# jjhbw/GoMILP

Measured on AMD Instinct MI355X. Metric: simplex pivots/sec on 2048x4096 fp64 dense LP, higher is better.
Workload: dtype f64

## Files before the change

gomilp_amd/csrc/lu_cross.hip:

```cpp
#include <hip/hip_runtime.h>
#include <stdint.h>

#include "bt_loop.h"
#include "device_types.h"
#include "kernels_common.h"
#include "luc_role.h"

namespace gomilp {

namespace {

constexpr int kLxSlots = 24;
constexpr int kLxSlots32 = 40;
constexpr int kLxHeader = 16;
constexpr int kLxSpinLimit = 400000;

__device__ __forceinline__ void lx_load3(const xpair *p0, const xpair *p1, const xpair *p2, xpair (&v)[3]) {
    asm volatile("global_load_dwordx4 %0, %3, off sc1\n\tglobal_load_dwordx4 %1, %4, off sc1\n\tglobal_load_dwordx4 %2, %5, off sc1\n\ts_waitcnt vmcnt(0)"
                 : "=&v"(v[0]), "=&v"(v[1]), "=&v"(v[2]) : "v"(p0), "v"(p1), "v"(p2) : "memory");
}

__device__ __forceinline__ void lx_load3_fast(const xpair *p0, const xpair *p1, const xpair *p2, xpair (&v)[3]) {
    asm volatile("global_load_dwordx4 %0, %3, off nt\n\tglobal_load_dwordx4 %1, %4, off nt\n\tglobal_load_dwordx4 %2, %5, off nt\n\ts_waitcnt vmcnt(0)"
                 : "=&v"(v[0]), "=&v"(v[1]), "=&v"(v[2]) : "v"(p0), "v"(p1), "v"(p2) : "memory");
}

__device__ __forceinline__ void lx_load5(const xpair *p, xpair (&v)[5]) {
    asm volatile("global_load_dwordx4 %0, %5, off sc1\n\tglobal_load_dwordx4 %1, %5, off offset:128 sc1\n\tglobal_load_dwordx4 %2, %5, off offset:256 sc1\n\t"
                 "global_load_dwordx4 %3, %5, off offset:384 sc1\n\tglobal_load_dwordx4 %4, %5, off offset:512 sc1\n\ts_waitcnt vmcnt(0)"
                 : "=&v"(v[0]), "=&v"(v[1]), "=&v"(v[2]), "=&v"(v[3]), "=&v"(v[4]) : "v"(p) : "memory");
}
__device__ __forceinline__ void lx_load5_fast(const xpair *p, xpair (&v)[5]) {
    asm volatile("global_load_dwordx4 %0, %5, off nt\n\tglobal_load_dwordx4 %1, %5, off offset:128 nt\n\tglobal_load_dwordx4 %2, %5, off offset:256 nt\n\t"
                 "global_load_dwordx4 %3, %5, off offset:384 nt\n\tglobal_load_dwordx4 %4, %5, off offset:512 nt\n\ts_waitcnt vmcnt(0)"
                 : "=&v"(v[0]), "=&v"(v[1]), "=&v"(v[2]), "=&v"(v[3]), "=&v"(v[4]) : "v"(p) : "memory");
}

}

#ifdef GOMILP_DEBUG
__device__ unsigned long long g_lux_stamps[4 * 16];
#define LUX_STAMP(S)                                                                      \
    do {                                                                                  \
        unsigned long long t_;                                                            \
        __builtin_amdgcn_sched_barrier(0);                                                \
        asm volatile("s_memtime %0\n\ts_waitcnt lgkmcnt(0)" : "=s"(t_)::"memory");        \
        __builtin_amdgcn_sched_barrier(0);                                                \
        if ((S) >= 0) tacc[(S) >= 0 ? (S) : 0] += t_ - tprev;                             \
        tprev = t_;                                                                       \
    } while (0)
#else
#define LUX_STAMP(S) do { } while (0)
#endif

template <int G, int RPT, int NB, int SMAX, bool LK>
__global__ __launch_bounds__(256) void k_luc_panel_x(LUArgs a, int32_t *__restrict__ pivrow, xpair *__restrict__ xrec) {
    constexpr int T = 256, NW = 4, MAXM = 256 * RPT * G;
    static_assert((NB == 16 || NB == 32) && SMAX <= 32 && G <= 8, "register tuples of 16 slots; lane l polls record l >> 3");
    static_assert(RPT == 1 || ((RPT == 4 || RPT == 8) && G == 8), "several rows per lane: the eight-workgroup panel");
    static_assert(!LK || RPT == 1, "the look-ahead role: one row per lane");
    static_assert(RPT < 8 || NB == 16, "eight rows per lane: one tuple of 16 slots");
    static_assert(MAXM <= 16384, "rows below 16384 fit (cnt << 16) | row in redL");
    constexpr bool KEEPX = RPT <= 4;
    constexpr int NH = NB / 16;
    constexpr int NSL = NB == 16 ? kLxSlots : kLxSlots32;
    constexpr int NLD = NSL / 8;
    constexpr int NUSE = 5 + NB;
    typedef unsigned short idx_t;
    typedef double vec __attribute__((ext_vector_type(16)));
    constexpr idx_t NONE = 0xFFFF;
    const int bx = (int)blockIdx.x;
    if ((bx & 7) || (bx >> 3) >= G) {
        if constexpr (LK) {
            if (!a.ctl_base->fault) luc_role<T, SMAX, true>(a, bx - min(G, (bx + 7) >> 3), (int)gridDim.x - G);
        }
        return;
    }
    const int g = bx >> 3;
    __shared__ idx_t s_lpos[MAXM];
    __shared__ idx_t s_rowat[MAXM];
    __shared__ idx_t s_unit[MAXM];
    __shared__ idx_t s_ucol[MAXM];
    __shared__ unsigned char s_active[MAXM];
    __shared__ double redM[2][NW];
    __shared__ unsigned int redL[2][NW];
    __shared__ int s_slotcol[NB];
    __shared__ int s_nload, s_stop, s_limit, s_sigma;
    __shared__ __attribute__((aligned(16))) double s_post[NW][NSL];
    if (a.ctl_base->fault) return;
    LUCtl *ctl = a.ctl;
    const int tid = threadIdx.x, lane = tid & 63, w = tid >> 6;
    const int m = a.m;
    const size_t ldw = (size_t)a.ldw;
    const int k0 = a.ctl_prev->k_next;
    if (k0 >= m) {
        if (g == 0 && tid == 0) luc_ctl_empty(ctl, a.ctl_prev, k0, true);
        return;
    }
#ifdef GOMILP_DEBUG
    unsigned long long tacc[16] = {}, tprev = 0;
#endif
    LUX_STAMP(-1);
    for (int R = tid; R < MAXM; R += T) {
        const bool in = R < m;
        s_lpos[R] = (idx_t)(in ? a.lpos[R] : R);
        s_active[R] = (in && a.rowstep[R] < 0) ? 1 : 0;
        const int ur = (in && a.unit_row) ? a.unit_row[R] : -1;
        s_unit[R] = ur < 0 ? NONE : (idx_t)ur;
        s_ucol[R] = NONE;
    }
    __syncthreads();
    for (int R = tid; R < m; R += T) {
        s_rowat[s_lpos[R]] = (idx_t)R;
        if (s_unit[R] != NONE && R >= k0) s_ucol[s_unit[R]] = (idx_t)R;
    }
    for (;;) {
        __syncthreads();
        bool again = false;
        for (int R = tid; R < m; R += T)
            if (s_unit[R] != NONE && R >= k0 && R < (int)s_ucol[s_unit[R]]) { s_ucol[s_unit[R]] = (idx_t)R; again = true; }
        if (!__syncthreads_or(again)) break;
    }
    if (w == 0) {
        const int n = luc_scan_dense<NB>(k0, m, s_unit, s_active, s_slotcol);
        if (lane == 0) s_nload = n;
    }
    __syncthreads();
    const int nload = s_nload;
    int myslotcol = (lane < NB && lane < nload) ? s_slotcol[lane < NB ? lane : 0] : 0x7FFFFFFF;
    int myslotin = -1;
    unsigned int live = nload >= 32 ? 0xFFFFFFFFu : ((1u << nload) - 1u);
    const int R0 = g * (T * RPT) + tid;
    bool act[RPT];
    int myucol[RPT];
#pragma unroll
    for (int r = 0; r < RPT; r++) {
        const int R = R0 + T * r;
        act[r] = (R < m) && s_active[R < m ? R : 0];
        const idx_t uc0 = s_ucol[R < m ? R : 0];
        myucol[r] = (act[r] && uc0 != NONE) ? (int)uc0 : 0x7FFFFFFF;
    }
    LUX_STAMP(9);
    if constexpr (LK) {
        if (tid == 0) s_stop = luc_spin(&a.ctl_base->cnt_u, (uint32_t)(a.round + 1) * (uint32_t)((m + 63) / 64)) ? 1 : 0;
        __syncthreads();
        if (!s_stop) {
            if (tid == 0) {
                a.ctl_base->fault = 1;
                if (g == 0) luc_ctl_empty(ctl, a.ctl_prev, k0, true);
            }
            return;
        }
    }
    LUX_STAMP(10);
    vec v[RPT][NH];
#pragma unroll
    for (int r = 0; r < RPT; r++) {
        const double *src = a.W + (act[r] ? R0 + T * r : 0);
        if constexpr (LK) {
#pragma unroll
            for (int c = 0; c < NB; c++) v[r][c / 16][c % 16] = (act[r] && c < nload) ? luc_ld_agent(&src[(size_t)__builtin_amdgcn_readlane(myslotcol, c) * ldw]) : 0.0;
        } else {
#pragma unroll
            for (int c = 0; c < NB; c++) v[r][c / 16][c % 16] = (act[r] && c < nload) ? src[(size_t)__builtin_amdgcn_readlane(myslotcol, c) * ldw] : 0.0;
        }
    }
    __syncthreads();
    __builtin_amdgcn_s_waitcnt(0x0F70);
    unsigned int myxcc;
    asm volatile("s_getreg_b32 %0, hwreg(HW_REG_XCC_ID)" : "=s"(myxcc));
    myxcc &= 0xFu;
    bool fast = false;
    const double seq0 = xrec[0][0];
    xpair *recs = xrec + kLxHeader / 2;
    int nx = 0;
    LUX_STAMP(11);
    int kcur = k0, s = 0, k1 = m;
    int ksync = a.ctl_prev->ksync;
    bool fault = false;
#pragma unroll 1
    for (;;) {
        if (w == 0) {
            const unsigned int key = (lane < NB && ((live >> lane) & 1u)) ? (unsigned int)myslotcol : 0x7FFFFFFFu;
            unsigned int mn = row_min_u32(key);
            if constexpr (NB == 16) mn = (unsigned int)__builtin_amdgcn_readlane((int)mn, 0);
            else mn = min((unsigned int)__builtin_amdgcn_readlane((int)mn, 0), (unsigned int)__builtin_amdgcn_readlane((int)mn, 16));
            const bool listed = live != 0 && s < SMAX;
            const int limit = listed ? (int)mn : m;
            const unsigned long long hit = __ballot(key == mn && lane < NB);
            const int sigma = hit ? (int)__builtin_ctzll(hit) : 0;
            int k = kcur;
            for (;;) {
                const int kk = k + lane;
                const idx_t ur = kk < limit ? s_unit[kk] : NONE;
                const bool triv = ur != NONE && s_active[ur] && (int)s_ucol[ur] == kk;
                const unsigned long long nt = __ballot(!triv);
                const int cnt = nt ? (int)__builtin_ctzll(nt) : 64;
                k += cnt;
                if (cnt < 64) break;
            }
            if (lane == 0) { s_stop = k; s_limit = limit; s_sigma = sigma; }
        }
        LUX_STAMP(0);
        __syncthreads();
        LUX_STAMP(1);
        const int kstop = s_stop, limit = s_limit;
        const int sigma = __builtin_amdgcn_readfirstlane(s_sigma) & (NB - 1);
        for (int c = kcur + tid; c < kstop; c += T) s_active[s_unit[c]] = 0;
#pragma unroll
        for (int r = 0; r < RPT; r++) {
            if (act[r] && myucol[r] >= kcur && myucol[r] < kstop) {
                const int R = R0 + T * r, kt = myucol[r];
                a.rowstep[R] = kt; pivrow[kt] = R;
                double *dst = a.W + R;
#pragma unroll
                for (int c = 0; c < NB; c++)
                    if ((live >> c) & 1u) dst[(size_t)__builtin_amdgcn_readlane(myslotcol, c) * ldw] = v[r][c / 16][c % 16];
                act[r] = false;
            }
        }
        if (kstop < limit || live == 0 || s >= SMAX) { k1 = kstop; break; }
        const int k = limit;
        LUX_STAMP(2);
        double xk[KEEPX ? RPT : 1];
        if constexpr (KEEPX) {
#pragma unroll
            for (int r = 0; r < RPT; r++) {
                if constexpr (NH == 1) xk[r] = v[r][0][sigma];
                else {
                    if (sigma < 16) { asm volatile(""); xk[r] = v[r][0][sigma & 15]; }
                    else { asm volatile(""); xk[r] = v[r][NH - 1][sigma & 15]; }
                }
            }
        }
        auto xof = [&](int r) -> double { if constexpr (KEEPX) return xk[r]; else return v[r][0][sigma]; };
        auto xmof = [&](int r) -> double { return act[r] ? -fabs(xof(r)) : __builtin_inf(); };
        double xml = __builtin_inf();
        if constexpr (RPT == 1) xml = xmof(0);
        else {
#pragma unroll
            for (int r = 0; r < RPT; r++) xml = fmin(xml, xmof(r));
        }
        xpair rv[NLD];
        auto exchange = [&](int pr, double h0, double h1) {
            const double seq = seq0 + (double)(nx + 1);
            xpair *mine = recs + ((size_t)((nx + 1) & 1) * G + g) * NSL;
            if (__any(pr >= 0)) {
                double *sp = s_post[w];
                if (pr >= 0) {
                    sp[0] = h0; sp[1] = h1;
#pragma unroll
                    for (int r = 0; r < RPT; r++) {
                        if (pr == r) {
                            sp[2] = (double)(R0 + T * r);
                            sp[3] = act[r] ? 1.0 / xof(r) : 0.0;
#pragma unroll
                            for (int c = 0; c < NB; c++) sp[4 + c] = v[r][c / 16][c % 16];
                        }
                    }
                    sp[4 + NB] = (double)myxcc;
                }
                __builtin_amdgcn_s_waitcnt(0xC07F);
                if (lane < NUSE) xstore(mine + lane, xpair{seq, sp[lane]}, fast);
            }
            const xpair *base = recs + (size_t)((nx + 1) & 1) * G * NSL;
            const int g2 = lane >> 3, j0 = lane & 7;
            const bool mineok = g2 < G;
            const xpair *q0 = base + (size_t)(mineok ? g2 : 0) * NSL + j0;
            for (int it = 0;; it++) {
                if constexpr (NLD == 3) { if (fast) lx_load3_fast(q0, q0 + 8, q0 + 16, rv); else lx_load3(q0, q0 + 8, q0 + 16, rv); }
                else { if (fast) lx_load5_fast(q0, rv); else lx_load5(q0, rv); }
                bool ok = true;
#pragma unroll
                for (int r = 0; r < NLD; r++) ok = ok && (j0 + 8 * r >= NUSE || rv[r][0] == seq);
                ok = ok || !mineok;
                if (__all(ok)) break;
                if (it >= kLxSpinLimit) { fault = true; break; }
                __builtin_amdgcn_s_sleep(1);
            }
            nx++;
        };
        const bool head = (lane & 7) == 0 && (lane >> 3) < G;
        const double wm = wave_min_f64(xml);
        unsigned int cntw = 0, lk = 0xFFFFFFFFu;
#pragma unroll
        for (int r = 0; r < RPT; r++) {
            const bool hit = act[r] && xmof(r) == wm;
            cntw += (unsigned int)__popcll(__ballot(hit));
            lk = min(lk, hit ? (unsigned int)(R0 + T * r) : 0xFFFFFFFFu);
        }
        lk = row_min_u32(lk);
        lk = min(min((unsigned int)__builtin_amdgcn_readlane((int)lk, 15), (unsigned int)__builtin_amdgcn_readlane((int)lk, 31)),
                 min((unsigned int)__builtin_amdgcn_readlane((int)lk, 47), (unsigned int)__builtin_amdgcn_readlane((int)lk, 63)));
        double *rm = redM[s & 1];
        unsigned int *rl = redL[s & 1];
        if (lane == 0) { rm[w] = wm; rl[w] = (min(cntw, 2u) << 16) | (lk & 0xFFFFu); }
        LUX_STAMP(3);
        __syncthreads();
        LUX_STAMP(4);
        const double bx = lane < NW ? rm[lane] : __builtin_inf();
        const double bml = readlane_f64(row_min_f64(bx), 15);
        const unsigned int infol = (lane < NW && bx == bml) ? rl[lane] : 0u;
        const unsigned int cntl = (unsigned int)__popcll(__ballot((infol >> 16) >= 1u)) + (unsigned int)__popcll(__ballot((infol >> 16) >= 2u));
        const unsigned int rowl = (unsigned int)__builtin_amdgcn_readlane((int)row_min_u32((lane < NW && (infol >> 16) >= 1u) ? (infol & 0xFFFFu) : 0xFFFFFFFFu), 15);
        int pr = -1;
        if (cntl) {
#pragma unroll
            for (int r = 0; r < RPT; r++) pr = (act[r] && (unsigned int)(R0 + T * r) == rowl) ? r : pr;
        } else if (tid == 0) pr = 0;
        exchange(pr, cntl ? bml : __builtin_inf(), (double)min(cntl, 2u));
        if (fault) break;
        LUX_STAMP(5);
        if (!fast) {
            const double xc = __shfl(rv[(4 + NB) >> 3][1], (lane & ~7) + 4);
            fast = __all(!head || xc == (double)myxcc);
        }
        const double wmL = head ? rv[0][1] : __builtin_inf();
        const double bm = wave_min_f64(wmL);
        const double cnL = __shfl(rv[0][1], (lane & ~7) + 1);
        const unsigned long long at1 = __ballot(head && wmL == bm && cnL >= 1.0), at2 = __ballot(head && wmL == bm && cnL >= 2.0);
        int gw;
        if (__popcll(at1) == 1 && at2 == 0) {
            gw = (int)__builtin_ctzll(at1) >> 3;
        } else {
            asm volatile("s_waitcnt vmcnt(0)" ::: "memory");
            __syncthreads();
            exchange(tid == 0 ? 0 : -1, 0.0, 0.0);
            if (fault) break;
            if (w == 0) {
                for (int j0 = ksync; j0 < k; j0 += 64) {
                    const int jj = j0 + lane;
                    const int pj = jj < k ? __hip_atomic_load(&pivrow[jj], __ATOMIC_RELAXED, __HIP_MEMORY_SCOPE_AGENT) : 0;
                    const int nrep = min(64, k - j0);
                    for (int t = 0; t < nrep; t++) {
                        const int Pj = __builtin_amdgcn_readlane(pj, t);
                        if (lane == 0) {
                            const idx_t jq = s_lpos[Pj], Q = s_rowat[j0 + t];
                            s_lpos[Q] = jq; s_rowat[jq] = Q;
                            s_lpos[Pj] = (idx_t)(j0 + t); s_rowat[j0 + t] = (idx_t)Pj;
                        }
                    }
                }
            }
            ksync = k;
            __syncthreads();
            unsigned int lpmine = 0xFFFFFFFFu;
            int rmine = 0;
#pragma unroll
            for (int r = 0; r < RPT; r++) {
                const bool tied = act[r] && xmof(r) == bm;
                const unsigned int lpr = tied ? (unsigned int)s_lpos[tied ? R0 + T * r : 0] : 0xFFFFFFFFu;
                rmine = lpr < lpmine ? r : rmine;
                lpmine = min(lpmine, lpr);
            }
            unsigned int lp = row_min_u32(lpmine);
            lp = min(min((unsigned int)__builtin_amdgcn_readlane((int)lp, 15), (unsigned int)__builtin_amdgcn_readlane((int)lp, 31)),
                     min((unsigned int)__builtin_amdgcn_readlane((int)lp, 47), (unsigned int)__builtin_amdgcn_readlane((int)lp, 63)));
            unsigned int *rt = redL[(s & 1) ^ 1];
            if (lane == 0) rt[w] = lp;
            __syncthreads();
            const unsigned int lpl = (unsigned int)__builtin_amdgcn_readlane((int)row_min_u32(lane < NW ? rt[lane] : 0xFFFFFFFFu), 15);
            const bool any_l = lpl != 0xFFFFFFFFu;
            exchange(any_l ? (lpmine == lpl ? rmine : -1) : (tid == 0 ? 0 : -1), any_l ? (double)lpl : __builtin_inf(), 0.0);
            if (fault) break;
            const double lpL = head ? rv[0][1] : __builtin_inf();
            const double blp = wave_min_f64(lpL);
            const unsigned long long won = __ballot(head && lpL == blp);
            gw = won ? ((int)__builtin_ctzll(won) >> 3) : 0;
        }
        const int P = (int)readlane_f64(rv[0][1], 8 * gw + 2);
        const double rinv = readlane_f64(rv[0][1], 8 * gw + 3);
        double prl;
        {
            const int c = lane & (NB - 1);
            const int src = 8 * gw + ((4 + c) & 7), rr = (4 + c) >> 3;
            prl = __shfl(rv[0][1], src);
#pragma unroll
            for (int r = 1; r < NLD; r++) {
                const double br = __shfl(rv[r][1], src);
                prl = rr == r ? br : prl;
            }
        }
        LUX_STAMP(6);
        if (tid == 0 && P >= 0 && P < MAXM) s_active[P] = 0;
#pragma unroll
        for (int r = 0; r < RPT; r++) {
            if (act[r] && R0 + T * r == P) {
                act[r] = false;
                a.rowstep[P] = k; pivrow[k] = P;
                if (a.dense_flag) a.dense_flag[k] = 1;
                ctl->steps[s] = k; ctl->prow[s] = P;
                double *dst = a.W + (R0 + T * r);
#pragma unroll
                for (int cc = 0; cc < NB; cc++)
                    if ((live >> cc) & 1u) dst[(size_t)__builtin_amdgcn_readlane(myslotcol, cc) * ldw] = v[r][cc / 16][cc % 16];
                if (readlane_f64(prl, sigma) == 0) a.st->lu_singular = 1;
            }
        }
        const idx_t uc = (P >= 0 && P < MAXM) ? s_ucol[P] : NONE;
        const int k2 = (uc != NONE && (int)uc > k) ? (int)uc : -1;
        LUX_STAMP(7);
        const double piv = readlane_f64(prl, sigma);
        const bool singular = (piv == 0);
        double *wcol = a.W + (size_t)k * ldw;
        double *lcol = a.Lp + (size_t)s * ldw;
        const unsigned int others = live & ~(1u << sigma);
        const double prz = (lane < NB && ((others >> (lane & 31)) & 1u)) ? prl : 0.0;
#pragma unroll
        for (int r = 0; r < RPT; r++) {
            const int R = R0 + T * r;
            double nl = 0.0;
            if (act[r]) {
                const double xr = xof(r);
                const double l = singular ? xr : __dmul_rn(xr, rinv);
                wcol[R] = l;
                nl = singular ? 0.0 : -l;
                lcol[R] = nl;
            } else if (R < a.ldw) lcol[R] = 0.0;
            if (!singular && __any(act[r])) {
#pragma unroll
                for (int c = 0; c < NB; c++) {
                    const double pc = readlane_f64(prz, c);
                    v[r][c / 16][c % 16] = __dadd_rn(__dmul_rn(nl, pc), v[r][c / 16][c % 16]);
                }
            }
            if (k2 >= 0) {
                const double vn = (act[r] && !singular) ? __dadd_rn(__dmul_rn(nl, 1.0), 0.0) : 0.0;
                if constexpr (NH == 1) { asm volatile(""); v[r][0][sigma] = vn; }
                else {
                    if (sigma < 16) { asm volatile(""); v[r][0][sigma & 15] = vn; }
                    else { asm volatile(""); v[r][NH - 1][sigma & 15] = vn; }
                }
            }
        }
        if (k2 >= 0) {
            if (lane == sigma) { myslotcol = k2; myslotin = k; }
        } else live = others;
        s++;
        kcur = k + 1;
        LUX_STAMP(8);
    }
    if (fault) {
        if (lane == 0) a.ctl_base->fault = 1;
        return;
    }
    if constexpr (LK) {
#pragma unroll
        for (int r = 0; r < RPT; r++) {
            const int R = R0 + T * r;
            if (R < m) a.rowsnap[R] = act[r] ? -1 : a.rowstep[R];
        }
    }
    if (g != 0) return;
    __syncthreads();
    for (int R2 = tid; R2 < m; R2 += T) a.lpos[R2] = s_lpos[R2];
    int ndl = 0;
    if (w == 0) {
        if constexpr (LK) {
            const int n = luc_scan_dense<NB>(k1, m, s_unit, s_active, ctl->next);
            if (lane == 0) ctl->nnext = n;
        } else if (lane == 0) ctl->nnext = 0;
        const bool on = lane < NB && ((live >> lane) & 1u);
        const unsigned long long msk = __ballot(on);
        ndl = __popcll(msk);
        if (on) {
            const int at = __popcll(msk & ((1ull << lane) - 1ull));
            ctl->dropcol[at] = myslotcol; ctl->dropin[at] = myslotin; ctl->dropout[at] = k1;
        }
    }
    if (tid == 0) {
        ctl->k0 = k0; ctl->k1 = k1; ctl->k_next = k1; ctl->nsteps = s; ctl->ndrop = ndl;
        ctl->rounds = a.ctl_prev->rounds + 1; ctl->ksync = ksync;
        xrec[0] = xpair{seq0 + (double)nx, 0.0};
    }
    LUX_STAMP(12);
#ifdef GOMILP_DEBUG
    if (lane == 0) {
        for (int sg = 0; sg < 13; sg++) atomicAdd(&g_lux_stamps[w * 16 + sg], tacc[sg]);
        if (w == 0) { atomicAdd(&g_lux_stamps[15], (unsigned long long)s); atomicAdd(&g_lux_stamps[14], 1ull); }
    }
#endif
}

__global__ void k_luc_lpos_final(LUArgs a) {
    const int R = blockIdx.x * blockDim.x + threadIdx.x;
    if (R < a.m) a.lpos[R] = a.rowstep[R];
}
void launch_luc_lpos_final(const LUArgs &a, hipStream_t s) { hipLaunchKernelGGL(k_luc_lpos_final, dim3((a.m + 255) / 256), dim3(256), 0, s, a); }

size_t luc_cross_doubles() { return (size_t)kLxHeader + 2 * 2 * 8 * kLxSlots32; }
int luc_cross_groups(int m, int want) {
    if (want <= 0 || m < 64) return 0;
    const int need = (m + 255) / 256;
    if (need > 8) return 0;
    return need <= 2 ? 2 : (need <= 4 ? 4 : 8);
}
int luc_large_rpt(int m) { return (m <= 4096 || m > 16384) ? 0 : (m <= 8192 ? 4 : 8); }
template <int G, int RPT>
static void luc_cross_panel(const LUArgs &a, int32_t *pivrow, double *xrec, int slots, int nrole, hipStream_t s) {
    xpair *xr = reinterpret_cast<xpair *>(xrec);
    constexpr bool look = RPT == 1 && G >= 4;
    if (slots != 32 || RPT == 8) hipLaunchKernelGGL((k_luc_panel_x<G, RPT, 16, 32, false>), dim3(8 * G), dim3(256), 0, s, a, pivrow, xr);
    else if constexpr (RPT < 8) {
        if (nrole <= 0 || !look) hipLaunchKernelGGL((k_luc_panel_x<G, RPT, 32, 32, false>), dim3(8 * G), dim3(256), 0, s, a, pivrow, xr);
        else if constexpr (look) hipLaunchKernelGGL((k_luc_panel_x<G, 1, 32, 32, true>), dim3(G + (nrole > 8 * G ? nrole : 8 * G)), dim3(256), 0, s, a, pivrow, xr);
    }
}
void launch_luc_cross_panel(const LUArgs &a, int32_t *pivrow, double *xrec, int G, int slots, int nrole, hipStream_t s) {
    const int rpt = luc_large_rpt(a.m);
    if (rpt == 8) luc_cross_panel<8, 8>(a, pivrow, xrec, slots, nrole, s);
    else if (rpt == 4) luc_cross_panel<8, 4>(a, pivrow, xrec, slots, nrole, s);
    else if (G == 2) luc_cross_panel<2, 1>(a, pivrow, xrec, slots, nrole, s);
    else if (G == 4) luc_cross_panel<4, 1>(a, pivrow, xrec, slots, nrole, s);
    else luc_cross_panel<8, 1>(a, pivrow, xrec, slots, nrole, s);
}
#ifdef GOMILP_DEBUG
void lux_stamps_read(unsigned long long *out) { (void)hipMemcpyFromSymbol(out, HIP_SYMBOL(g_lux_stamps), sizeof(unsigned long long) * 64); }
#endif

}
```

Baseline: 241,400.

## Overlap next-column search and retired-row stores with cross-workgroup exchange polling

For the one-row-per-lane panel, the next pivot column and trivial-run end are computed speculatively inside the exchange, after the poll loads are issued and before waiting on them. This removes a per-step wave-0 scan and a __syncthreads from the critical path. Stores of retired rows are deferred and issued just before the poll loads so they overlap the exchange latency, with a final flush after the loop. The speculative limit and sigma are patched when a new column enters. This adds complexity and ordering risk around s_active updates and deferred stores. The look-ahead spin also uses __syncthreads_or instead of a shared flag.

```diff
diff --git a/gomilp_amd/csrc/lu_cross.hip b/gomilp_amd/csrc/lu_cross.hip
--- a/gomilp_amd/csrc/lu_cross.hip
+++ b/gomilp_amd/csrc/lu_cross.hip
@@ -14,6 +14,10 @@
 constexpr int kLxSlots32 = 40;
 constexpr int kLxHeader = 16;
 constexpr int kLxSpinLimit = 400000;
+#ifndef GOMILP_LUX_STORES_UNDER_POLL
+#define GOMILP_LUX_STORES_UNDER_POLL 1
+#endif
+constexpr bool kLxStoresUnderPoll = GOMILP_LUX_STORES_UNDER_POLL != 0;
 
 __device__ __forceinline__ void lx_load3(const xpair *p0, const xpair *p1, const xpair *p2, xpair (&v)[3]) {
     asm volatile("global_load_dwordx4 %0, %3, off sc1\n\tglobal_load_dwordx4 %1, %4, off sc1\n\tglobal_load_dwordx4 %2, %5, off sc1\n\ts_waitcnt vmcnt(0)"
@@ -35,6 +39,23 @@
                  "global_load_dwordx4 %3, %5, off offset:384 nt\n\tglobal_load_dwordx4 %4, %5, off offset:512 nt\n\ts_waitcnt vmcnt(0)"
                  : "=&v"(v[0]), "=&v"(v[1]), "=&v"(v[2]), "=&v"(v[3]), "=&v"(v[4]) : "v"(p) : "memory");
 }
+
+__device__ __forceinline__ void lx_issue3(const xpair *p0, const xpair *p1, const xpair *p2, xpair (&v)[3], bool fast) {
+    if (fast) asm volatile("global_load_dwordx4 %0, %3, off nt\n\tglobal_load_dwordx4 %1, %4, off nt\n\tglobal_load_dwordx4 %2, %5, off nt"
+                           : "=&v"(v[0]), "=&v"(v[1]), "=&v"(v[2]) : "v"(p0), "v"(p1), "v"(p2) : "memory");
+    else asm volatile("global_load_dwordx4 %0, %3, off sc1\n\tglobal_load_dwordx4 %1, %4, off sc1\n\tglobal_load_dwordx4 %2, %5, off sc1"
+                      : "=&v"(v[0]), "=&v"(v[1]), "=&v"(v[2]) : "v"(p0), "v"(p1), "v"(p2) : "memory");
+}
+__device__ __forceinline__ void lx_issue5(const xpair *p, xpair (&v)[5], bool fast) {
+    if (fast) asm volatile("global_load_dwordx4 %0, %5, off nt\n\tglobal_load_dwordx4 %1, %5, off offset:128 nt\n\tglobal_load_dwordx4 %2, %5, off offset:256 nt\n\t"
+                           "global_load_dwordx4 %3, %5, off offset:384 nt\n\tglobal_load_dwordx4 %4, %5, off offset:512 nt"
+                           : "=&v"(v[0]), "=&v"(v[1]), "=&v"(v[2]), "=&v"(v[3]), "=&v"(v[4]) : "v"(p) : "memory");
+    else asm volatile("global_load_dwordx4 %0, %5, off sc1\n\tglobal_load_dwordx4 %1, %5, off offset:128 sc1\n\tglobal_load_dwordx4 %2, %5, off offset:256 sc1\n\t"
+                      "global_load_dwordx4 %3, %5, off offset:384 sc1\n\tglobal_load_dwordx4 %4, %5, off offset:512 sc1"
+                      : "=&v"(v[0]), "=&v"(v[1]), "=&v"(v[2]), "=&v"(v[3]), "=&v"(v[4]) : "v"(p) : "memory");
+}
+__device__ __forceinline__ void lx_wait(xpair (&v)[3]) { asm volatile("s_waitcnt vmcnt(0)" : "+v"(v[0]), "+v"(v[1]), "+v"(v[2]) : : "memory"); }
+__device__ __forceinline__ void lx_wait(xpair (&v)[5]) { asm volatile("s_waitcnt vmcnt(0)" : "+v"(v[0]), "+v"(v[1]), "+v"(v[2]), "+v"(v[3]), "+v"(v[4]) : : "memory"); }
 
 }
 
@@ -61,6 +82,8 @@
     static_assert(!LK || RPT == 1, "the look-ahead role: one row per lane");
     static_assert(RPT < 8 || NB == 16, "eight rows per lane: one tuple of 16 slots");
     static_assert(MAXM <= 16384, "rows below 16384 fit (cnt << 16) | row in redL");
+    constexpr bool AHEAD = RPT == 1;
+    constexpr bool STORES_LATE = AHEAD && kLxStoresUnderPoll;
     constexpr bool KEEPX = RPT <= 4;
     constexpr int NH = NB / 16;
     constexpr int NSL = NB == 16 ? kLxSlots : kLxSlots32;
@@ -142,9 +165,8 @@
     }
     LUX_STAMP(9);
     if constexpr (LK) {
-        if (tid == 0) s_stop = luc_spin(&a.ctl_base->cnt_u, (uint32_t)(a.round + 1) * (uint32_t)((m + 63) / 64)) ? 1 : 0;
-        __syncthreads();
-        if (!s_stop) {
+        const bool come = tid == 0 && luc_spin(&a.ctl_base->cnt_u, (uint32_t)(a.round + 1) * (uint32_t)((m + 63) / 64));
+        if (!__syncthreads_or(come ? 1 : 0)) {
             if (tid == 0) {
                 a.ctl_base->fault = 1;
                 if (g == 0) luc_ctl_empty(ctl, a.ctl_prev, k0, true);
@@ -178,50 +200,91 @@
     int kcur = k0, s = 0, k1 = m;
     int ksync = a.ctl_prev->ksync;
     bool fault = false;
+    auto next_col = [&](unsigned int lv, int sn, int &lim, int &sg) {
+        const unsigned int key = (lane < NB && ((lv >> lane) & 1u)) ? (unsigned int)myslotcol : 0x7FFFFFFFu;
+        unsigned int mn = row_min_u32(key);
+        if constexpr (NB == 16) mn = (unsigned int)__builtin_amdgcn_readlane((int)mn, 0);
+        else mn = min((unsigned int)__builtin_amdgcn_readlane((int)mn, 0), (unsigned int)__builtin_amdgcn_readlane((int)mn, 16));
+        lim = (lv != 0 && sn < SMAX) ? (int)mn : m;
+        const unsigned long long hit = __ballot(key == mn && lane < NB);
+        sg = hit ? (int)__builtin_ctzll(hit) : 0;
+    };
+    auto run_end = [&](int from, int lim) -> int {
+        int k = from;
+        for (;;) {
+            const int kk = k + lane;
+            const idx_t ur = kk < lim ? s_unit[kk] : NONE;
+            const bool triv = ur != NONE && s_active[ur] && (int)s_ucol[ur] == kk;
+            const unsigned long long nt = __ballot(!triv);
+            const int cnt = nt ? (int)__builtin_ctzll(nt) : 64;
+            k += cnt;
+            if (cnt < 64) break;
+        }
+        return k;
+    };
+    auto store_row = [&](int r) {
+        double *dst = a.W + (R0 + T * r);
+#pragma unroll
+        for (int c = 0; c < NB; c++)
+            if ((live >> c) & 1u) dst[(size_t)__builtin_amdgcn_readlane(myslotcol, c) * ldw] = v[r][c / 16][c % 16];
+    };
+    auto retired = [&](int r, int ke) -> bool { return myucol[r] >= kcur && myucol[r] < ke; };
+    int limit_c = m, sigma_c = 0, kstop_c = k0;
+    if constexpr (AHEAD) {
+        next_col(live, 0, limit_c, sigma_c);
+        kstop_c = run_end(k0, limit_c);
+    }
 #pragma unroll 1
     for (;;) {
-        if (w == 0) {
-            const unsigned int key = (lane < NB && ((live >> lane) & 1u)) ? (unsigned int)myslotcol : 0x7FFFFFFFu;
-            unsigned int mn = row_min_u32(key);
-            if constexpr (NB == 16) mn = (unsigned int)__builtin_amdgcn_readlane((int)mn, 0);
-            else mn = min((unsigned int)__builtin_amdgcn_readlane((int)mn, 0), (unsigned int)__builtin_amdgcn_readlane((int)mn, 16));
-            const bool listed = live != 0 && s < SMAX;
-            const int limit = listed ? (int)mn : m;
-            const unsigned long long hit = __ballot(key == mn && lane < NB);
-            const int sigma = hit ? (int)__builtin_ctzll(hit) : 0;
-            int k = kcur;
-            for (;;) {
-                const int kk = k + lane;
-                const idx_t ur = kk < limit ? s_unit[kk] : NONE;
-                const bool triv = ur != NONE && s_active[ur] && (int)s_ucol[ur] == kk;
-                const unsigned long long nt = __ballot(!triv);
-                const int cnt = nt ? (int)__builtin_ctzll(nt) : 64;
-                k += cnt;
-                if (cnt < 64) break;
-            }
-            if (lane == 0) { s_stop = k; s_limit = limit; s_sigma = sigma; }
-        }
-        LUX_STAMP(0);
-        __syncthreads();
-        LUX_STAMP(1);
-        const int kstop = s_stop, limit = s_limit;
-        const int sigma = __builtin_amdgcn_readfirstlane(s_sigma) & (NB - 1);
-        for (int c = kcur + tid; c < kstop; c += T) s_active[s_unit[c]] = 0;
+        int kstop, limit, sigma;
+        if constexpr (AHEAD) { kstop = kstop_c; limit = limit_c; sigma = sigma_c & (NB - 1); }
+        else {
+            if (w == 0) {
+                const unsigned int key = (lane < NB && ((live >> lane) & 1u)) ? (unsigned int)myslotcol : 0x7FFFFFFFu;
+                unsigned int mn = row_min_u32(key);
+                if constexpr (NB == 16) mn = (unsigned int)__builtin_amdgcn_readlane((int)mn, 0);
+                else mn = min((unsigned int)__builtin_amdgcn_readlane((int)mn, 0), (unsigned int)__builtin_amdgcn_readlane((int)mn, 16));
+                const bool listed = live != 0 && s < SMAX;
+                const int lim = listed ? (int)mn : m;
+                const unsigned long long hit = __ballot(key == mn && lane < NB);
+                const int sg = hit ? (int)__builtin_ctzll(hit) : 0;
+                int ke = kcur;
+                for (;;) {
+                    const int kk = ke + lane;
+                    const idx_t ur = kk < lim ? s_unit[kk] : NONE;
+                    const bool triv = ur != NONE && s_active[ur] && (int)s_ucol[ur] == kk;
+                    const unsigned long long nt = __ballot(!triv);
+                    const int cnt = nt ? (int)__builtin_ctzll(nt) : 64;
+                    ke += cnt;
+                    if (cnt < 64) break;
+                }
+                if (lane == 0) { s_stop = ke; s_limit = lim; s_sigma = sg; }
+            }
+            LUX_STAMP(0);
+            __syncthreads();
+            LUX_STAMP(1);
+            kstop = s_stop; limit = s_limit;
+            sigma = __builtin_amdgcn_readfirstlane(s_sigma) & (NB - 1);
+            for (int c = kcur + tid; c < kstop; c += T) s_active[s_unit[c]] = 0;
+        }
 #pragma unroll
         for (int r = 0; r < RPT; r++) {
             if (act[r] && myucol[r] >= kcur && myucol[r] < kstop) {
                 const int R = R0 + T * r, kt = myucol[r];
                 a.rowstep[R] = kt; pivrow[kt] = R;
-                double *dst = a.W + R;
-#pragma unroll
-                for (int c = 0; c < NB; c++)
-                    if ((live >> c) & 1u) dst[(size_t)__builtin_amdgcn_readlane(myslotcol, c) * ldw] = v[r][c / 16][c % 16];
+                if constexpr (!STORES_LATE) {
+                    double *dst = a.W + R;
+#pragma unroll
+                    for (int c = 0; c < NB; c++)
+                        if ((live >> c) & 1u) dst[(size_t)__builtin_amdgcn_readlane(myslotcol, c) * ldw] = v[r][c / 16][c % 16];
+                }
                 act[r] = false;
             }
         }
         if (kstop < limit || live == 0 || s >= SMAX) { k1 = kstop; break; }
         const int k = limit;
-        LUX_STAMP(2);
+        if constexpr (AHEAD) LUX_STAMP(0);
+        else LUX_STAMP(2);
         double xk[KEEPX ? RPT : 1];
         if constexpr (KEEPX) {
 #pragma unroll
@@ -242,7 +305,7 @@
             for (int r = 0; r < RPT; r++) xml = fmin(xml, xmof(r));
         }
         xpair rv[NLD];
-        auto exchange = [&](int pr, double h0, double h1) {
+        auto exchange = [&](int pr, double h0, double h1, auto &&stores, auto &&under) {
             const double seq = seq0 + (double)(nx + 1);
             xpair *mine = recs + ((size_t)((nx + 1) & 1) * G + g) * NSL;
             if (__any(pr >= 0)) {
@@ -267,9 +330,20 @@
             const int g2 = lane >> 3, j0 = lane & 7;
             const bool mineok = g2 < G;
             const xpair *q0 = base + (size_t)(mineok ? g2 : 0) * NSL + j0;
+            if constexpr (AHEAD) {
+                LUX_STAMP(2);
+                stores();
+                if constexpr (NLD == 3) lx_issue3(q0, q0 + 8, q0 + 16, rv, fast);
+                else lx_issue5(q0, rv, fast);
+                under();
+                LUX_STAMP(1);
+                lx_wait(rv);
+            }
             for (int it = 0;; it++) {
-                if constexpr (NLD == 3) { if (fast) lx_load3_fast(q0, q0 + 8, q0 + 16, rv); else lx_load3(q0, q0 + 8, q0 + 16, rv); }
-                else { if (fast) lx_load5_fast(q0, rv); else lx_load5(q0, rv); }
+                if (!AHEAD || it > 0) {
+                    if constexpr (NLD == 3) { if (fast) lx_load3_fast(q0, q0 + 8, q0 + 16, rv); else lx_load3(q0, q0 + 8, q0 + 16, rv); }
+                    else { if (fast) lx_load5_fast(q0, rv); else lx_load5(q0, rv); }
+                }
                 bool ok = true;
 #pragma unroll
                 for (int r = 0; r < NLD; r++) ok = ok && (j0 + 8 * r >= NUSE || rv[r][0] == seq);
@@ -308,7 +382,20 @@
 #pragma unroll
             for (int r = 0; r < RPT; r++) pr = (act[r] && (unsigned int)(R0 + T * r) == rowl) ? r : pr;
         } else if (tid == 0) pr = 0;
-        exchange(pr, cntl ? bml : __builtin_inf(), (double)min(cntl, 2u));
+        int limit_n = 0, sigma_n = 0, kstop_n = 0;
+        exchange(pr, cntl ? bml : __builtin_inf(), (double)min(cntl, 2u), [&]() {
+            if constexpr (STORES_LATE) {
+#pragma unroll
+                for (int r = 0; r < RPT; r++)
+                    if (retired(r, kstop)) store_row(r);
+            }
+        }, [&]() {
+            if constexpr (AHEAD) {
+                for (int c = kcur + tid; c < kstop; c += T) s_active[s_unit[c]] = 0;
+                next_col(live & ~(1u << sigma), s + 1, limit_n, sigma_n);
+                kstop_n = run_end(k + 1, limit_n);
+            }
+        });
         if (fault) break;
         LUX_STAMP(5);
         if (!fast) {
@@ -325,7 +412,7 @@
         } else {
             asm volatile("s_waitcnt vmcnt(0)" ::: "memory");
             __syncthreads();
-            exchange(tid == 0 ? 0 : -1, 0.0, 0.0);
+            exchange(tid == 0 ? 0 : -1, 0.0, 0.0, []() {}, []() {});
             if (fault) break;
             if (w == 0) {
                 for (int j0 = ksync; j0 < k; j0 += 64) {
@@ -361,7 +448,7 @@
             __syncthreads();
             const unsigned int lpl = (unsigned int)__builtin_amdgcn_readlane((int)row_min_u32(lane < NW ? rt[lane] : 0xFFFFFFFFu), 15);
             const bool any_l = lpl != 0xFFFFFFFFu;
-            exchange(any_l ? (lpmine == lpl ? rmine : -1) : (tid == 0 ? 0 : -1), any_l ? (double)lpl : __builtin_inf(), 0.0);
+            exchange(any_l ? (lpmine == lpl ? rmine : -1) : (tid == 0 ? 0 : -1), any_l ? (double)lpl : __builtin_inf(), 0.0, []() {}, []() {});
             if (fault) break;
             const double lpL = head ? rv[0][1] : __builtin_inf();
             const double blp = wave_min_f64(lpL);
@@ -435,15 +522,28 @@
         }
         if (k2 >= 0) {
             if (lane == sigma) { myslotcol = k2; myslotin = k; }
+            if constexpr (AHEAD) {
+                if (s + 1 < SMAX) {
+                    sigma_n = k2 < limit_n ? sigma : sigma_n;
+                    limit_n = min(limit_n, k2);
+                }
+                kstop_n = min(kstop_n, k2);
+            }
         } else live = others;
         s++;
         kcur = k + 1;
+        if constexpr (AHEAD) { limit_c = limit_n; sigma_c = sigma_n; kstop_c = kstop_n; }
         LUX_STAMP(8);
     }
     if (fault) {
         if (lane == 0) a.ctl_base->fault = 1;
         return;
     }
+    if constexpr (STORES_LATE) {
+#pragma unroll
+        for (int r = 0; r < RPT; r++)
+            if (retired(r, k1)) store_row(r);
+    }
     if constexpr (LK) {
 #pragma unroll
         for (int r = 0; r < RPT; r++) {
@@ -452,6 +552,10 @@
         }
     }
     if (g != 0) return;
+    if constexpr (AHEAD) {
+        __syncthreads();
+        for (int c = kcur + tid; c < k1; c += T) s_active[s_unit[c]] = 0;
+    }
     __syncthreads();
     for (int R2 = tid; R2 < m; R2 += T) a.lpos[R2] = s_lpos[R2];
     int ndl = 0;
```

New measurement: 242,100, median of 3. No clear change (+0.3%).
